# MadNLP/MadNLP.jl

Measured on NVIDIA H100. Metric: ipm_iters_per_sec, higher is better.
Workload: dtype f64

## Files before the change

### include/b200kkt.h

```cpp
#ifndef B200KKT_H
#define B200KKT_H

#include <stdint.h>

#ifdef __cplusplus
extern "C" {
#endif

#define B2_OK                 0
#define B2_ERR_INVALID        1
#define B2_ERR_CUDA           2
#define B2_ERR_SYMBOLIC       3
#define B2_ERR_FACTORIZATION  4
#define B2_ERR_SOLVE          5
#define B2_ERR_NO_DEVICE      6
#define B2_ERR_UNSUPPORTED    7

#define B2_ORDER_METIS_ND 0
#define B2_ORDER_MINDEG   1
#define B2_ORDER_NATURAL  2
#define B2_ORDER_USER     3

const char* b2_last_error(void);
int b2_version(void);
// ... 3 lines not shown
    int32_t ordering;
    int32_t nemin;
    double  relax_zeros;
    double  pivot_eps;
    int32_t use_cuda_graph;
    int32_t small_front_max;
    int32_t n_parts;
    int32_t part_rank;
    int32_t kkt_n_primal;
    int32_t fuse_max_fronts;
    int32_t dep_schedule;
    int32_t chain_merge_f;
    int32_t kkt_n_dual;
    int32_t dense_pivoting;
    int32_t sparse_pivoting;
    int32_t reserved[1];
} b2_options;

#define B2_DENSE_PIVOT_STATIC        0
#define B2_DENSE_PIVOT_BUNCH_KAUFMAN 1
#define B2_SPARSE_PIVOT_STATIC       0
#define B2_SPARSE_PIVOT_PAIRS        1

#define B2_PIVOT_1X1            0
#define B2_PIVOT_1X1_PERTURBED  1
#define B2_PIVOT_2X2_FIRST      2
#define B2_PIVOT_2X2_SECOND     3

int b2_options_default(b2_options* opt);

typedef struct b2_solver b2_solver;

typedef struct b2_stats {
    int64_t n, nnz_a, nnz_l, flops;
    int64_t n_supernodes, n_levels;
    int64_t max_front, n_small_fronts, n_big_fronts;
    int64_t factor_bytes, workspace_bytes;
    int64_t sep_rows;
    int64_t n_factor_launches, n_solve_launches;
    int64_t n_perturbed;
} b2_stats;

int b2_create(int32_t n, int64_t nnz, const int32_t* colptr_h, const int32_t* rowval_h,
              const double* nzval_d, const b2_options* opt, const int32_t* user_perm_h,
              b2_solver** out);
int b2_create_symbolic_only(int32_t n, int64_t nnz, const int32_t* colptr_h, const int32_t* rowval_h,
                            const b2_options* opt, const int32_t* user_perm_h, b2_solver** out);
int b2_destroy(b2_solver* s);
int b2_set_values_ptr(b2_solver* s, const double* nzval_d);
int b2_factorize(b2_solver* s, void* stream);
int b2_inertia(b2_solver* s, int64_t* num_pos, int64_t* num_zero, int64_t* num_neg, void* stream);
int b2_inertia_enqueue(b2_solver* s, void* stream);
int b2_inertia_fetch(b2_solver* s, int64_t* num_pos, int64_t* num_zero, int64_t* num_neg);
int b2_solve(b2_solver* s, double* x_d, int32_t nrhs, void* stream);
int b2_improve(b2_solver* s, int32_t* changed);
int b2_get_stats(b2_solver* s, b2_stats* st);
int b2_get_perm(b2_solver* s, int32_t* perm_h);

int b2_exchange_buffer(b2_solver* s, double** buf_d, int64_t* n_factor_doubles, int64_t* n_solve_doubles);
int b2_exchange_vector(b2_solver* s, double** buf_d, int64_t* n_doubles);
int b2_inertia_parts(b2_solver* s, int64_t* local_neg, int64_t* local_zero, int64_t* top_neg, int64_t* top_zero, void* stream);
int b2_factorize_local(b2_solver* s, void* stream);
int b2_factorize_top(b2_solver* s, void* stream);
int b2_solve_fwd_local(b2_solver* s, double* x_d, void* stream);
int b2_solve_top(b2_solver* s, double* x_d, void* stream);
int b2_solve_bwd_local(b2_solver* s, double* x_d, void* stream);
int b2_owned_mask(b2_solver* s, uint8_t* owned_h);

typedef struct b2_symbolic_sizes {
    int64_t n, n_supernodes, n_rows, n_children, n_rel, n_amap, n_levels, lval_size, cb_size;
} b2_symbolic_sizes;
int b2_symbolic_query(b2_solver* s, b2_symbolic_sizes* sz);
int b2_symbolic_export(b2_solver* s, int32_t* perm, int32_t* sn_first, int32_t* sn_parent, int32_t* sn_level,
                       int64_t* rows_ptr, int32_t* rows, int64_t* lp_off, int64_t* cb_off,
                       int64_t* rel_ptr, int32_t* rel, int64_t* amap_ptr, int64_t* amap_src, int64_t* amap_dst);
int b2_symbolic_owner(b2_solver* s, int32_t* owner);
int b2_symbolic_exchange(b2_solver* s, int64_t* cbv_off, int64_t* exch_cb, int64_t* exch_cbv);
int b2_debug_get_factor(b2_solver* s, double* lval_h, double* dvec_h);
int b2_symbolic_pairs(b2_solver* s, uint8_t* pair_start_h);
int b2_get_pivot_blocks(b2_solver* s, int8_t* kind_h, double* d_h, double* d_off_h);
int b2_debug_profile_front(b2_solver* s, int32_t sn, int32_t reps, int64_t* stamps_h);
int b2_debug_trace(b2_solver* s, uint64_t* stamps_h, int32_t* parent_h, int32_t* w_h, int32_t* f_h, int64_t capacity, int64_t* count);
int b2_debug_trace_solve(b2_solver* s, uint64_t* stamps_h, int64_t capacity, int64_t* count);

typedef struct b2d_solver b2d_solver;
int b2d_create(int32_t N, int32_t lda, const double* A_d, const b2_options* opt, b2d_solver** out);
int b2d_destroy(b2d_solver* s);
int b2d_debug_trace(b2d_solver* s, uint64_t* stamps_h, int64_t capacity, int64_t* count);
int b2d_factorize(b2d_solver* s, void* stream);
int b2d_inertia(b2d_solver* s, int64_t* num_pos, int64_t* num_zero, int64_t* num_neg, void* stream);
int b2d_inertia_enqueue(b2d_solver* s, void* stream);
int b2d_inertia_fetch(b2d_solver* s, int64_t* num_pos, int64_t* num_zero, int64_t* num_neg);
int b2d_solve(b2d_solver* s, double* x_d, int32_t nrhs, void* stream);
int b2d_get_pivots(b2d_solver* s, int32_t* ipiv_h, double* d_h, double* e_h);

int b2_coo_to_csc(int32_t m, int32_t n, int64_t nnz_coo, const int32_t* I_h, const int32_t* J_h,
                  int32_t* colptr_h, int32_t* rowval_h, int64_t* map_h, int64_t* nnz_csc);

int b2_coo_to_csc_device(int32_t m, int32_t n, int64_t nnz_coo, const int32_t* I_d, const int32_t* J_d,
                         int32_t* colptr_d, int32_t* rowval_d, int64_t* map_d, int64_t* nnz_csc, void* stream);

typedef struct b2_transfer_plan b2_transfer_plan;
int b2_transfer_plan_create(int64_t nnz_coo, int64_t nnz_csc, const int64_t* map_h, b2_transfer_plan** out);
int b2_transfer_plan_destroy(b2_transfer_plan* p);
int b2_transfer(b2_transfer_plan* p, double* dst_nz_d, const double* V_d, void* stream);

typedef struct b2_condensed_plan b2_condensed_plan;
int b2_condensed_symbolic(int32_t n, int32_t m,
                          const int32_t* H_colptr_h, const int32_t* H_rowval_h,
                          const int32_t* Jt_colptr_h, const int32_t* Jt_rowval_h,
                          b2_condensed_plan** out, int64_t* nnz_aug);
int b2_condensed_symbolic_device(int32_t n, int32_t m,
                                 const int32_t* H_colptr_d, const int32_t* H_rowval_d,
                                 const int32_t* Jt_colptr_d, const int32_t* Jt_rowval_d,
                                 b2_condensed_plan** out, int64_t* nnz_aug, void* stream);
int b2_condensed_pattern(b2_condensed_plan* p, int32_t* colptr_h, int32_t* rowval_h);
int b2_condensed_plan_sizes(b2_condensed_plan* p, int64_t* n_dptr, int64_t* n_hptr, int64_t* n_jptr);
int b2_condensed_plan_destroy(b2_condensed_plan* p);
int b2_condensed_assemble(b2_condensed_plan* p, double* aug_nz_d, const double* pr_diag_d,
                          const double* du_diag_d, const double* H_nz_d, const double* Jt_nz_d,
                          double* diag_buffer_d, void* stream);

int b2d_condensed_assemble(int32_t n, int32_t m, int32_t ns, int32_t n_eq,
                           const int64_t* ind_ineq_d, const int64_t* ind_eq_d,
                           const double* hess_d, const double* jac_d,
                           const double* pr_diag_d, const double* du_diag_d,
                           double* diag_buffer_d, double* aug_d, void* stream);

int b2d_aug_assemble(int32_t n, int32_t m, int32_t ns, const int64_t* ind_ineq_d,
                     const double* hess_d, const double* jac_d, const double* pr_diag_d,
                     const double* du_diag_d, const double* diag_hess_d, double* aug_d, void* stream);
int b2d_copy_diag(int32_t n, int32_t lda, const double* A_d, double* d_d, void* stream);

typedef struct b2d_ozaki_plan b2d_ozaki_plan;
int b2d_ozaki_plan_create(int32_t n, int32_t ns, b2d_ozaki_plan** out);
int b2d_ozaki_plan_destroy(b2d_ozaki_plan* p);
int b2d_condensed_assemble_ozaki(b2d_ozaki_plan* p, int32_t n, int32_t m, int32_t ns, int32_t n_eq,
                                 const int64_t* ind_ineq_d, const int64_t* ind_eq_d,
                                 const double* hess_d, const double* jac_d,
                                 const double* pr_diag_d, const double* du_diag_d,
                                 double* diag_buffer_d, double* aug_d, void* stream);
int b2d_ozaki_plan_status(b2d_ozaki_plan* p, int32_t* timed_out, void* stream);

int b2d_gemv_n(int32_t rows, int32_t cols, int32_t lda, const double* A_d, const double* x_d, double* y_d, double alpha, double beta, void* stream);
int b2d_gemv_t(int32_t rows, int32_t cols, int32_t lda, const double* A_d, const double* x_d, double* y_d, double alpha, double beta, void* stream);
int b2d_symv_lower(int32_t n, int32_t lda, const double* A_d, const double* x_d, double* y_d, double alpha, double beta, void* stream);

typedef struct b2_bounds b2_bounds;
typedef struct b2d_kkt b2d_kkt;
int b2d_kkt_create(int32_t n, int32_t m, int32_t ns, const int64_t* ind_ineq_h, b2d_kkt** out);
int b2d_kkt_destroy(b2d_kkt* k);
int b2d_kkt_solve_pre(b2d_kkt* k, b2_bounds* b, const double* jac_d, const double* pr_diag_d, const double* diag_buffer_d,
                      const double* l_diag_d, const double* u_diag_d, double* buffer_d, double* pd_buffer_d, double* w_d, void* stream);
int b2d_kkt_solve_post(b2d_kkt* k, b2_bounds* b, const double* jac_d, const double* pr_diag_d, const double* diag_buffer_d,
                       const double* l_lower_d, const double* u_lower_d, const double* l_diag_d, const double* u_diag_d,
                       const double* buffer_d, const double* pd_buffer_d, double* w_d, void* stream);
int b2d_kkt_mul(b2d_kkt* k, b2_bounds* b, const double* hess_d, const double* jac_d, const double* reg_d, const double* du_diag_d,
                const double* l_lower_d, const double* u_lower_d, const double* l_diag_d, const double* u_diag_d,
                double alpha, double beta, const double* x_d, double* w_d, void* stream);

typedef struct b2_bounds b2_bounds;
int b2_bounds_create(int64_t n_tot, int64_t nlb, int64_t nub, const int64_t* ind_lb_h, const int64_t* ind_ub_h,
                     b2_bounds** out);
int b2_bounds_destroy(b2_bounds* b);

int b2_set_aug_diagonal(b2_bounds* b, const double* reg_d, const double* l_lower_d, const double* l_diag_d,
// ... 307 lines not shown
```

### madnlp.jl_b200/capi.py

```python
from __future__ import annotations

import ctypes as C
import os

_HERE = os.path.dirname(os.path.abspath(__file__))
LIB_PATH = os.path.join(_HERE, "csrc", "libb200kkt.so")

B2_OK = 0
B2_ERR_INVALID, B2_ERR_CUDA, B2_ERR_SYMBOLIC, B2_ERR_FACTORIZATION, B2_ERR_SOLVE, B2_ERR_NO_DEVICE, B2_ERR_UNSUPPORTED = 1, 2, 3, 4, 5, 6, 7
ORDER_METIS_ND, ORDER_MINDEG, ORDER_NATURAL, ORDER_USER = 0, 1, 2, 3
QN_BFGS, QN_DAMPED_BFGS = 1, 2
B2_DENSE_PIVOT_STATIC, B2_DENSE_PIVOT_BUNCH_KAUFMAN = 0, 1
B2_SPARSE_PIVOT_STATIC, B2_SPARSE_PIVOT_PAIRS = 0, 1
B2_PIVOT_1X1, B2_PIVOT_1X1_PERTURBED, B2_PIVOT_2X2_FIRST, B2_PIVOT_2X2_SECOND = 0, 1, 2, 3
CURV_WXT, CURV_WXN, CURV_GN, CURV_TT, CURV_LHS, CURV_PASS, CURV_RESULT_LEN = 0, 1, 2, 3, 4, 5, 6
DUAL_INIT_NORM, DUAL_INIT_COPY, DUAL_INIT_RESULT_LEN = 0, 1, 2
QF_TAU, QF_NRM_PRIMAL, QF_NRM_DUAL, QF_MU_AVG, QF_SCAL_LEN = 0, 1, 2, 3, 4
QF_SIGMA, QF_MU, QF_N_EVAL, QF_N_GS_ITER, QF_TOL_EXIT, QF_TRACE, QF_MAX_GS_ITER = 0, 1, 2, 3, 4, 8, 64
KRYLOV_MAX_RESTART, KRYLOV_Y, KRYLOV_REC, KRYLOV_REC_LEN, KRYLOV_STATE_LEN = 16, 321, 344, 8, 352
KREC_EST, KREC_H, KREC_NORM_W, KREC_NORM_X, KREC_NORM_B, KREC_NORM_B2 = 0, 1, 2, 3, 4, 5


def qf_result_len(max_gs_iter):
    return QF_TRACE + 4 * (6 + max_gs_iter)
# ... 50 lines not shown


class InertiaSource(C.Structure):
    _fields_ = [("counters_d", C.c_void_p), ("n", C.c_int64), ("neg", C.c_int32 * 2), ("zero", C.c_int32 * 2), ("fail", C.c_int32),
                ("reserved", C.c_int32)]


class RefineRecord(C.Structure):
    _fields_ = [("ratio", C.c_double), ("norm_w", C.c_double), ("norm_x", C.c_double), ("norm_b", C.c_double), ("ir", C.c_int64),
                ("steps", C.c_int64), ("num_pos", C.c_int64), ("num_zero", C.c_int64), ("num_neg", C.c_int64), ("inertia_ok", C.c_int32),
                ("fail", C.c_int32), ("seq", C.c_int64)]


class InertiaSchedule(C.Structure):
    _fields_ = [(k, C.c_double) for k in ("first_hessian_perturbation", "min_hessian_perturbation", "max_hessian_perturbation",
                                          "perturb_inc_fact_first", "perturb_inc_fact", "perturb_dec_fact")]


TRIALS_ACCEPTED, TRIALS_FAILED, TRIALS_HANDOVER, TRIALS_FAULT = 1, 2, 3, 4


class InertiaRecord(C.Structure):
    _fields_ = [("status", C.c_int32), ("inertia_ok", C.c_int32), ("trials", C.c_int64), ("del_w", C.c_double),
                ("del_w_prev", C.c_double), ("del_c_prev", C.c_double), ("num_pos", C.c_int64), ("num_zero", C.c_int64),
                ("num_neg", C.c_int64), ("ir", C.c_int64), ("ratio", C.c_double), ("ir_total", C.c_int64), ("seq", C.c_int64)]


class SymbolicSizes(C.Structure):
    _fields_ = [(k, C.c_int64) for k in (
        "n", "n_supernodes", "n_rows", "n_children", "n_rel", "n_amap", "n_levels", "lval_size", "cb_size")]


def _load():
    if not os.path.exists(LIB_PATH):
        raise ImportError(
            f"{LIB_PATH} not found: build it with `python -c 'import __graft_entry__ as g; g.build()'` "
            f"(or `make -C madnlp.jl_b200/csrc`). The GPU KKT path has no CPU fallback.")
    return C.CDLL(LIB_PATH)


lib = _load()

_p = C.c_void_p
_i32, _i64, _f64 = C.c_int32, C.c_int64, C.c_double
_PP = C.POINTER(C.c_void_p)

PROTOTYPES = {
    "b2_last_error": (C.c_char_p, []),
    "b2_version": (C.c_int, []),
    "b2_device_count": (C.c_int, [C.POINTER(C.c_int)]),
    "b2_options_default": (C.c_int, [C.POINTER(Options)]),
    "b2_create": (C.c_int, [_i32, _i64, _p, _p, _p, C.POINTER(Options), _p, _PP]),
    "b2_create_symbolic_only": (C.c_int, [_i32, _i64, _p, _p, C.POINTER(Options), _p, _PP]),
    "b2_destroy": (C.c_int, [_p]),
    "b2_set_values_ptr": (C.c_int, [_p, _p]),
    "b2_factorize": (C.c_int, [_p, _p]),
    "b2_inertia": (C.c_int, [_p, C.POINTER(_i64), C.POINTER(_i64), C.POINTER(_i64), _p]),
    "b2_inertia_enqueue": (C.c_int, [_p, _p]),
    "b2_inertia_fetch": (C.c_int, [_p, C.POINTER(_i64), C.POINTER(_i64), C.POINTER(_i64)]),
    "b2_solve": (C.c_int, [_p, _p, _i32, _p]),
    "b2_improve": (C.c_int, [_p, C.POINTER(_i32)]),
    "b2_get_stats": (C.c_int, [_p, C.POINTER(Stats)]),
    "b2_get_perm": (C.c_int, [_p, _p]),
    "b2_exchange_buffer": (C.c_int, [_p, _PP, C.POINTER(_i64), C.POINTER(_i64)]),
    "b2_exchange_vector": (C.c_int, [_p, _PP, C.POINTER(_i64)]),
    "b2_inertia_parts": (C.c_int, [_p, C.POINTER(_i64), C.POINTER(_i64), C.POINTER(_i64), C.POINTER(_i64), _p]),
    "b2_factorize_local": (C.c_int, [_p, _p]),
    "b2_factorize_top": (C.c_int, [_p, _p]),
    "b2_solve_fwd_local": (C.c_int, [_p, _p, _p]),
    "b2_solve_top": (C.c_int, [_p, _p, _p]),
    "b2_solve_bwd_local": (C.c_int, [_p, _p, _p]),
    "b2_owned_mask": (C.c_int, [_p, _p]),
    "b2_symbolic_query": (C.c_int, [_p, C.POINTER(SymbolicSizes)]),
    "b2_symbolic_export": (C.c_int, [_p] + [_p] * 13),
    "b2_symbolic_owner": (C.c_int, [_p, _p]),
    "b2_symbolic_exchange": (C.c_int, [_p, _p, C.POINTER(_i64), C.POINTER(_i64)]),
    "b2_debug_get_factor": (C.c_int, [_p, _p, _p]),
    "b2_symbolic_pairs": (C.c_int, [_p, _p]),
    "b2_get_pivot_blocks": (C.c_int, [_p, _p, _p, _p]),
    "b2_debug_profile_front": (C.c_int, [_p, _i32, _i32, _p]),
    "b2d_debug_trace": (C.c_int, [_p, _p, _i64, C.POINTER(_i64)]),
    "b2_debug_trace": (C.c_int, [_p, _p, _p, _p, _p, _i64, C.POINTER(_i64)]),
    "b2_debug_trace_solve": (C.c_int, [_p, _p, _i64, C.POINTER(_i64)]),
    "b2d_create": (C.c_int, [_i32, _i32, _p, C.POINTER(Options), _PP]),
    "b2d_destroy": (C.c_int, [_p]),
    "b2d_factorize": (C.c_int, [_p, _p]),
    "b2d_inertia": (C.c_int, [_p, C.POINTER(_i64), C.POINTER(_i64), C.POINTER(_i64), _p]),
    "b2d_inertia_enqueue": (C.c_int, [_p, _p]),
    "b2d_inertia_fetch": (C.c_int, [_p, C.POINTER(_i64), C.POINTER(_i64), C.POINTER(_i64)]),
    "b2d_solve": (C.c_int, [_p, _p, _i32, _p]),
    "b2d_get_pivots": (C.c_int, [_p, _p, _p, _p]),
    "b2_condensed_symbolic_device": (C.c_int, [_i32, _i32, _p, _p, _p, _p, _PP, C.POINTER(_i64), _p]),
    "b2_coo_to_csc_device": (C.c_int, [_i32, _i32, _i64, _p, _p, _p, _p, _p, C.POINTER(_i64), _p]),
    "b2d_ozaki_plan_create": (C.c_int, [_i32, _i32, _PP]),
    "b2d_ozaki_plan_destroy": (C.c_int, [_p]),
    "b2d_condensed_assemble_ozaki": (C.c_int, [_p, _i32, _i32, _i32, _i32] + [_p] * 9),
    "b2d_ozaki_plan_status": (C.c_int, [_p, C.POINTER(_i32), _p]),
    "b2d_kkt_create": (C.c_int, [_i32, _i32, _i32, _p, _PP]),
    "b2d_kkt_destroy": (C.c_int, [_p]),
    "b2d_kkt_solve_pre": (C.c_int, [_p] * 10 + [_p]),
    "b2d_kkt_solve_post": (C.c_int, [_p] * 12 + [_p]),
    "b2d_kkt_mul": (C.c_int, [_p] * 10 + [_f64, _f64, _p, _p, _p]),
    "b2d_gemv_n": (C.c_int, [_i32, _i32, _i32, _p, _p, _p, _f64, _f64, _p]),
    "b2d_gemv_t": (C.c_int, [_i32, _i32, _i32, _p, _p, _p, _f64, _f64, _p]),
    "b2d_symv_lower": (C.c_int, [_i32, _i32, _p, _p, _p, _f64, _f64, _p]),
    "b2_coo_to_csc": (C.c_int, [_i32, _i32, _i64, _p, _p, _p, _p, _p, C.POINTER(_i64)]),
    "b2_transfer_plan_create": (C.c_int, [_i64, _i64, _p, _PP]),
    "b2_transfer_plan_destroy": (C.c_int, [_p]),
    "b2_transfer": (C.c_int, [_p, _p, _p, _p]),
    "b2_condensed_symbolic": (C.c_int, [_i32, _i32, _p, _p, _p, _p, _PP, C.POINTER(_i64)]),
    "b2_condensed_pattern": (C.c_int, [_p, _p, _p]),
    "b2_condensed_plan_sizes": (C.c_int, [_p, C.POINTER(_i64), C.POINTER(_i64), C.POINTER(_i64)]),
    "b2_condensed_plan_destroy": (C.c_int, [_p]),
    "b2_condensed_assemble": (C.c_int, [_p, _p, _p, _p, _p, _p, _p, _p]),
    "b2d_condensed_assemble": (C.c_int, [_i32, _i32, _i32, _i32, _p, _p, _p, _p, _p, _p, _p, _p, _p]),
    "b2d_aug_assemble": (C.c_int, [_i32, _i32, _i32] + [_p] * 8),
    "b2d_copy_diag": (C.c_int, [_i32, _i32, _p, _p, _p]),
    "b2_bounds_create": (C.c_int, [_i64, _i64, _i64, _p, _p, _PP]),
    "b2_bounds_destroy": (C.c_int, [_p]),
    "b2_set_aug_diagonal": (C.c_int, [_p, _p, _p, _p, _p, _p, _p, _p]),
    "b2_set_aug_diagonal_unreduced": (C.c_int, [_i64, _i64, _i64] + [_p] * 7),
    "b2_unreduced_solve_pre": (C.c_int, [_i64, _i64, _i64, _i64, _p, _p, _p, _p]),
    "b2_unreduced_solve_post": (C.c_int, [_i64, _i64, _i64, _i64, _p, _p, _p, _p]),
    "b2_regularize_diagonal": (C.c_int, [_i64, _i64, _f64, _f64, _p, _p, _p, _p]),
    "b2_reduce_rhs": (C.c_int, [_p, _i64, _p, _p, _p, _p]),
    "b2_finish_aug_solve": (C.c_int, [_p, _i64, _p, _p, _p, _p, _p, _p]),
    "b2_spmv_plan_create": (C.c_int, [_i32, _i32, _p, _p, _PP]),
    "b2_spmv_plan_destroy": (C.c_int, [_p]),
    "b2_spmv_n": (C.c_int, [_p, _p, _p, _p, _f64, _f64, _p]),
    "b2_spmv_t": (C.c_int, [_p, _p, _p, _p, _f64, _f64, _p]),
    "b2_spmv_symlower": (C.c_int, [_p, _p, _p, _p, _f64, _f64, _p]),
    "b2_kktmul": (C.c_int, [_p, _i64, _p, _p, _p, _p, _p, _p, _f64, _f64, _p, _p, _p]),
    "b2_condensed_solve_pre": (C.c_int, [_p, _p, _i64, _i64, _p, _p, _p, _p, _p, _p, _p, _p]),
    "b2_condensed_solve_post": (C.c_int, [_p, _p, _i64, _i64, _p, _p, _p, _p, _p, _p, _p, _p, _p, _p]),
    "b2_condensed_kkt_mul": (C.c_int, [_p, _p, _p, _i64, _i64, _p, _p, _p, _p, _p, _p, _p, _p, _f64, _f64, _p, _p, _p]),
    "b2_condensed_kkt_mul_norm": (C.c_int, [_p, _p, _p, _i64, _i64, _p, _p, _p, _p, _p, _p, _p, _p, _f64, _f64, _p, _p, _p, _p]),
    "b2_condensed_refine_pre": (C.c_int, [_p, _p, _i64, _i64, _p, _p, _p, _p, _p, _p, _p, _p, _p]),
    "b2_condensed_solve_post_update": (C.c_int, [_p, _p, _i64, _i64, _p, _p, _p, _p, _p, _p, _p, _p, _p, _p, _p, _p]),
    "b2_condensed_kkt_mul_norm_y": (C.c_int, [_p, _p, _p, _i64, _i64, _p, _p, _p, _p, _p, _p, _p, _p, _f64, _f64, _p, _p, _p, _p, _p]),
    "b2_get_alpha_max": (C.c_int, [_p, _p, _p, _p, _p, _f64, _p, _p]),
    "b2_get_alpha_z": (C.c_int, [_p, _p, _p, _p, _p, _f64, _p, _p]),
    "b2_get_varphi": (C.c_int, [_p, _f64, _p, _p, _p, _f64, _p, _p]),
    "b2_get_varphi_d": (C.c_int, [_p, _p, _p, _p, _p, _p, _f64, _p, _p]),
    "b2_get_inf_du": (C.c_int, [_p, _p, _p, _p, _p, _f64, _p, _p]),
    "b2_get_inf_compl": (C.c_int, [_p, _p, _p, _p, _p, _p, _f64, _f64, _p, _p]),
    "b2_get_average_complementarity": (C.c_int, [_p, _p, _p, _p, _p, _p, _p, _p]),
    "b2_get_min_complementarity": (C.c_int, [_p, _p, _p, _p, _p, _p, _p, _p]),
    "b2_get_rel_search_norm": (C.c_int, [_p, _i64, _p, _p, _p, _p]),
    "b2_get_sd": (C.c_int, [_p, _i64, _p, _p, _p, _f64, _p, _p]),
    "b2_get_sc": (C.c_int, [_p, _p, _p, _f64, _p, _p]),
    "b2_set_aug_rhs": (C.c_int, [_p, _i64, _p, _p, _p, _p, _p, _p, _p, _p, _f64, _p, _p]),
    "b2_set_g_ifr": (C.c_int, [_i64, _p, _p, _p, _p, _p, _f64, _p, _p]),
    "b2_set_aug_rhs_ifr": (C.c_int, [_i64, _i64, _i64, _i64, _p, _p, _p]),
    "b2_mul_hess_blk_tail": (C.c_int, [_p, _i64, _i32] + [_p] * 9 + [_f64, _p, _p]),
    "b2_rr_init": (C.c_int, [_p, _i64, _p, _p, _f64, _f64] + [_p] * 10 + [_p]),
    "b2_set_aug_rr": (C.c_int, [_p, _i64, _f64, _f64, _f64] + [_p] * 16 + [_p]),
    "b2_set_aug_rhs_rr": (C.c_int, [_p, _i64] + [_p] * 13 + [_f64, _f64, _p, _p]),
    "b2_finish_aug_solve_rr": (C.c_int, [_i64] + [_p] * 6 + [_f64, _f64] + [_p] * 4 + [_p]),
    "b2_set_f_rr": (C.c_int, [_i64, _f64, _p, _p, _p, _p, _p]),
    "b2_reset_bound_dual": (C.c_int, [_i64, _p, _p, _f64, _f64, _p]),
    "b2_reset_bound_dual_lu": (C.c_int, [_p] + [_p] * 5 + [_f64, _f64, _p]),
    "b2_adjust_boundary": (C.c_int, [_p, _p, _p, _p, _f64, _p]),
    "b2_get_theta": (C.c_int, [_p, _i64, _p, _p, _p]),
    "b2_get_theta_r": (C.c_int, [_p, _i64, _p, _p, _p, _p, _p]),
    "b2_get_inf_pr_r": (C.c_int, [_p, _i64, _p, _p, _p, _p, _p]),
    "b2_get_obj_val_r": (C.c_int, [_p, _i64] + [_p] * 5 + [_f64, _f64, _p, _p]),
# ... 129 lines not shown
```

### madnlp.jl_b200/csrc/sparse_ldl.cu

```cuda
#include <algorithm>
#include <cstdlib>
#include <cstring>
#include <stdexcept>
#include <vector>

#include "analysis.hpp"
#include "common.cuh"
#include "front_kernels.cuh"
#include "bigfactor_kernels.cuh"
#include "solve_kernels.cuh"
#include "warp_kernels.cuh"
#include "bigsolve_kernels.cuh"
#include "densesolve_kernels.cuh"
#include "dense_bk.cuh"

using namespace b2;

namespace {

struct WarpLaunch {
    int n_cta = 0, cta_ptr_off = 0, stage_off_off = 0, stage_cnt_off = 0;
    int nw = 1;
    int maxf = 0;
};
// ... 319 lines not shown
}

template <int NR>
constexpr size_t solve_block_smem() {
    return sizeof(double) * std::max<size_t>((size_t)4 * SolveSmem<1, NR>::doubles, (size_t)SolveSmem<2, NR>::doubles);
}
template <int NR>
const void* solve_block_kernel(bool pairs) {
    return pairs ? (const void*)k_solve_dep_block<NR, true> : (const void*)k_solve_dep_block<NR, false>;
}

template <int NR>
void enqueue_solve_block(b2_solver* s, double* x, int ncol, cudaStream_t st) {
    const Phase& P = s->phase[0];
    SolveArgs a = solve_args(s);
    a.perm = s->d_perm.p;
    a.x = x;
    const int64_t nr = s->cbv_off[s->S.nsuper];
    a.up = s->d_bslots.p;
    a.down = s->d_bslots.p + NR * nr;
    a.ypiv = s->d_bslots.p + 2 * NR * nr;
    DepSched ds;
    ds.grp_type = s->d_sched.p + P.dep_type_off; ds.grp_ptr = s->d_sched.p + P.dep_ptr_off; ds.tasks = s->d_sched.p + P.dep_tasks_off;
    ds.ngroup = P.dep_ngroup;
    const int w = NR == 2 ? 0 : NR == 4 ? 1 : 2;
    auto kern = s->pairs ? k_solve_dep_block<NR, true> : k_solve_dep_block<NR, false>;
    kern<<<P.sol_grid_blk[w], 128, solve_block_smem<NR>(), st>>>(a, s->d_childrec.p, ds, s->d_counters.p + 4, s->d_flags.p + s->S.nsuper + 1,
                                                                 s->S.n, ncol, s->d_bslots.p, (int64_t)s->d_bslots.n, s->d_dsub.p);
}

template <int NR>
cudaError_t set_level_block_attrs() {
    const void* k[] = {(const void*)k_fwd_warp2_block<1, SOLVE_FUSED_TEAMS, NR>, (const void*)k_bwd_warp2_block<1, SOLVE_FUSED_TEAMS, NR>,
                       (const void*)k_fwd_warp2_block<1, FW_WARPS, NR>, (const void*)k_bwd_warp2_block<1, FW_WARPS, NR>,
                       (const void*)k_fwd_warp2_block<2, 1, NR>, (const void*)k_bwd_warp2_block<2, 1, NR>,
                       (const void*)k_bs_head_block<NR>, (const void*)k_bs_fwd_block<NR>, (const void*)k_bs_bwd_block<NR>};
    for (const void* f : k) {
        cudaError_t e = cudaFuncSetAttribute(f, cudaFuncAttributeMaxDynamicSharedMemorySize, 100 * 1024);
        if (e != cudaSuccess) return e;
    }
    return cudaSuccess;
}

int set_smem_attrs() {
    B2_CUDA(cudaFuncSetAttribute(k_front_smem<512>, cudaFuncAttributeMaxDynamicSharedMemorySize, 227 * 1024));
    B2_CUDA(cudaFuncSetAttribute(k_factor_warp<1>, cudaFuncAttributeMaxDynamicSharedMemorySize, 160 * 1024));
    B2_CUDA(cudaFuncSetAttribute(k_factor_warp<2>, cudaFuncAttributeMaxDynamicSharedMemorySize, 160 * 1024));
    B2_CUDA(cudaFuncSetAttribute(k_factor_dep, cudaFuncAttributeMaxDynamicSharedMemorySize, 160 * 1024));
    B2_CUDA(cudaFuncSetAttribute(k_factor_dep_pairs, cudaFuncAttributeMaxDynamicSharedMemorySize, 160 * 1024));
    B2_CUDA(cudaFuncSetAttribute(k_fwd_warp2<1>, cudaFuncAttributeMaxDynamicSharedMemorySize, 100 * 1024));
    B2_CUDA(cudaFuncSetAttribute(k_bwd_warp2<1>, cudaFuncAttributeMaxDynamicSharedMemorySize, 100 * 1024));
    B2_CUDA(cudaFuncSetAttribute((k_fwd_warp2<1, SOLVE_FUSED_TEAMS>), cudaFuncAttributeMaxDynamicSharedMemorySize, 100 * 1024));
    B2_CUDA(cudaFuncSetAttribute((k_bwd_warp2<1, SOLVE_FUSED_TEAMS>), cudaFuncAttributeMaxDynamicSharedMemorySize, 100 * 1024));
    B2_CUDA(cudaFuncSetAttribute(k_fwd_warp2<2>, cudaFuncAttributeMaxDynamicSharedMemorySize, 100 * 1024));
    B2_CUDA(cudaFuncSetAttribute(k_bwd_warp2<2>, cudaFuncAttributeMaxDynamicSharedMemorySize, 100 * 1024));
    B2_CUDA(cudaFuncSetAttribute(k_solve_dep, cudaFuncAttributeMaxDynamicSharedMemorySize, 100 * 1024));
    B2_CUDA(cudaFuncSetAttribute(k_solve_dep_pairs, cudaFuncAttributeMaxDynamicSharedMemorySize, 100 * 1024));
    B2_CUDA(set_level_block_attrs<2>());
    B2_CUDA(set_level_block_attrs<4>());
    B2_CUDA(set_level_block_attrs<8>());
    for (bool pairs : {false, true}) {
        B2_CUDA(cudaFuncSetAttribute(solve_block_kernel<2>(pairs), cudaFuncAttributeMaxDynamicSharedMemorySize, 100 * 1024));
        B2_CUDA(cudaFuncSetAttribute(solve_block_kernel<4>(pairs), cudaFuncAttributeMaxDynamicSharedMemorySize, 100 * 1024));
        B2_CUDA(cudaFuncSetAttribute(solve_block_kernel<8>(pairs), cudaFuncAttributeMaxDynamicSharedMemorySize, 100 * 1024));
    }
    B2_CUDA(cudaFuncSetAttribute(k_big_inv, cudaFuncAttributeMaxDynamicSharedMemorySize, 160 * 1024));
    return B2_OK;
}

template <typename Fn>
int capture(b2_solver* s, cudaGraphExec_t* out, Fn fn) {
    if (*out) { cudaGraphExecDestroy(*out); *out = nullptr; }
    cudaGraph_t g = nullptr;
    B2_CUDA(cudaStreamBeginCapture(s->cap_stream, cudaStreamCaptureModeThreadLocal));
    fn(s->cap_stream);
    cudaError_t e = cudaStreamEndCapture(s->cap_stream, &g);
    if (e != cudaSuccess) return cuda_fail(e, "cudaStreamEndCapture", __FILE__, __LINE__);
    e = cudaGraphInstantiate(out, g, 0);
    cudaGraphDestroy(g);
    if (e != cudaSuccess) return cuda_fail(e, "cudaGraphInstantiate", __FILE__, __LINE__);
    return B2_OK;
}

void build_schedule(b2_solver* s) {
    const Symbolic& S = s->S;
    const int ns = S.nsuper;
    const int rank = std::max(0, s->opt.part_rank);
    const int smax = s->opt.small_front_max;
    const int wmax = std::min(W_MAX, smax);
    const int w1max = std::min(32, smax);
    const int fuse_max = s->opt.fuse_max_fronts;
    std::vector<int32_t> sched;
    auto fdim = [&](int sn, int& w, int& f) {
        w = S.sn_first[sn + 1] - S.sn_first[sn];
        f = (int)(S.rows_ptr[sn + 1] - S.rows_ptr[sn]);
    };
    auto emit_warp_launch = [&](const std::vector<std::vector<std::vector<int32_t>>>& ctas, int nw) {
        WarpLaunch L;
        L.nw = nw;
        L.n_cta = (int)ctas.size();
        std::vector<int32_t> cta_ptr(1, 0), st_off, st_cnt;
        for (const auto& stages : ctas) {
            for (const auto& fr : stages) {
                st_off.push_back((int32_t)sched.size());
                st_cnt.push_back((int32_t)fr.size());
                for (int32_t sn : fr) {
                    int w, f; fdim(sn, w, f);
                    L.maxf = std::max(L.maxf, f);
                    sched.push_back(sn);
                }
            }
            cta_ptr.push_back((int32_t)st_off.size());
        }
        L.cta_ptr_off = (int)sched.size(); sched.insert(sched.end(), cta_ptr.begin(), cta_ptr.end());
        L.stage_off_off = (int)sched.size(); sched.insert(sched.end(), st_off.begin(), st_off.end());
        L.stage_cnt_off = (int)sched.size(); sched.insert(sched.end(), st_cnt.begin(), st_cnt.end());
        return L;
    };
    for (int ph = 0; ph < 2; ++ph) {
        Phase& P = s->phase[ph];
        P.lev.clear(); P.fused = WarpLaunch(); P.n_fused_fronts = 0; P.dep_ngroup = 0; P.sol_grid = 0;
        std::vector<char> mine(ns, 0);
        for (int sn = 0; sn < ns; ++sn) mine[sn] = (ph == 0) ? (S.owner[sn] == rank) : (S.owner[sn] == -1);
        if ((s->opt.dep_schedule & 1) && s->opt.n_parts <= 1 && wmax > 32) {
            bool all_team = true;
            int cntm = 0;
            for (int sn = 0; sn < ns && all_team; ++sn) if (mine[sn]) { int w, f; fdim(sn, w, f); all_team = f <= wmax; ++cntm; }
            if (all_team && cntm > 0) {
                std::vector<int32_t> order;
                for (int l = 0; l < S.nlevels; ++l)
                    for (int q = S.level_ptr[l]; q < S.level_ptr[l + 1]; ++q) if (mine[S.level_sn[q]]) order.push_back(S.level_sn[q]);
                std::vector<int32_t> gtype, gptr(1, 0), tasks;
                size_t k = 0;
                while (k < order.size()) {
                    int w, f; fdim(order[k], w, f);
                    if (f > 32) {
                        gtype.push_back(2); tasks.push_back(order[k]); ++k;
                        P.dep_maxf2 = std::max(P.dep_maxf2, f);
                    } else {
                        gtype.push_back(1);
                        int c = 0;
                        while (k < order.size() && c < FW_WARPS) {
                            int w2, f2; fdim(order[k], w2, f2);
                            if (f2 > 32) break;
                            tasks.push_back(order[k]); P.dep_maxf1 = std::max(P.dep_maxf1, f2); ++k; ++c;
                        }
                    }
                    gptr.push_back((int32_t)tasks.size());
                }
                P.dep_ngroup = (int)gtype.size();
                P.dep_type_off = (int)sched.size(); sched.insert(sched.end(), gtype.begin(), gtype.end());
                P.dep_ptr_off = (int)sched.size(); sched.insert(sched.end(), gptr.begin(), gptr.end());
                P.dep_tasks_off = (int)sched.size(); sched.insert(sched.end(), tasks.begin(), tasks.end());
            }
        }
        std::vector<int32_t> cnt(ns, 0);
        std::vector<char> okw(ns, 0);
        for (int sn = 0; sn < ns; ++sn) {
            if (!mine[sn]) continue;
            int w, f; fdim(sn, w, f);
            bool ok = f <= w1max;
            int c = 1;
            for (int q = S.child_ptr[sn]; q < S.child_ptr[sn + 1]; ++q) {
                const int ch = S.child_idx[q];
                if (!mine[ch]) { continue; }
                ok = ok && okw[ch];
                c += cnt[ch];
            }
            cnt[sn] = c;
            okw[sn] = ok && fuse_max > 0 && c <= fuse_max;
        }
        std::vector<int32_t> root_of(ns, -1);
        std::vector<int32_t> roots;
        for (int sn = ns - 1; sn >= 0; --sn) {
            if (!mine[sn] || !okw[sn]) continue;
            const int p = S.sn_parent[sn];
            if (p >= 0 && mine[p] && okw[p]) root_of[sn] = root_of[p];
            else { root_of[sn] = sn; roots.push_back(sn); }
        }
        std::reverse(roots.begin(), roots.end());
        if (!roots.empty()) {
            std::vector<int32_t> ridx(ns, -1);
            for (size_t k = 0; k < roots.size(); ++k) ridx[roots[k]] = (int32_t)k;
            std::vector<std::vector<std::vector<int32_t>>> ctas(roots.size());
            for (int sn = 0; sn < ns; ++sn) {
                if (root_of[sn] < 0) continue;
                auto& stages = ctas[ridx[root_of[sn]]];
                const int lv = S.sn_level[sn];
                if ((int)stages.size() <= lv) stages.resize(lv + 1);
                stages[lv].push_back(sn);
                P.n_fused_fronts++;
            }
            for (auto& stages : ctas) {
                std::vector<std::vector<int32_t>> t;
                for (auto& v : stages) if (!v.empty()) t.push_back(std::move(v));
                stages.swap(t);
            }
            std::stable_sort(ctas.begin(), ctas.end(), [](const auto& a, const auto& b) {
                size_t na = 0, nb = 0;
                for (auto& v : a) na += v.size();
                for (auto& v : b) nb += v.size();
                return na > nb;
            });
            P.fused = emit_warp_launch(ctas, 1);
        }
        std::vector<int32_t> ulev(ns, -1);
        int nul = 0;
        for (int sn = 0; sn < ns; ++sn) {
            if (!mine[sn] || root_of[sn] >= 0) continue;
            int lv = 0;
            for (int q = S.child_ptr[sn]; q < S.child_ptr[sn + 1]; ++q) {
                const int ch = S.child_idx[q];
                if (mine[ch] && root_of[ch] < 0) lv = std::max(lv, ulev[ch] + 1);
            }
// ... 563 lines not shown
    return B2_OK;
}

int b2_exchange_buffer(b2_solver* s, double** buf_d, int64_t* n_factor_doubles, int64_t* n_solve_doubles) {
    if (!s || s->symbolic_only) return B2_ERR_INVALID;
    if (buf_d) *buf_d = s->d_ws.p;
    if (n_factor_doubles) *n_factor_doubles = s->S.exch_cb;
    if (n_solve_doubles) *n_solve_doubles = s->exch_cbv;
    return B2_OK;
}

int b2_exchange_vector(b2_solver* s, double** buf_d, int64_t* n_doubles) {
    if (!s || s->symbolic_only) return B2_ERR_INVALID;
    if (buf_d) *buf_d = s->d_cbv.p;
    if (n_doubles) *n_doubles = s->exch_cbv;
    return B2_OK;
}

int b2_owned_mask(b2_solver* s, uint8_t* owned_h) {
    if (!s || !owned_h) return B2_ERR_INVALID;
    std::memcpy(owned_h, s->owned_mask.data(), s->owned_mask.size());
    return B2_OK;
}

int b2_symbolic_query(b2_solver* s, b2_symbolic_sizes* sz) {
    if (!s || !sz) return B2_ERR_INVALID;
    const Symbolic& S = s->S;
    sz->n = S.n; sz->n_supernodes = S.nsuper; sz->n_rows = (int64_t)S.rows.size();
    sz->n_children = (int64_t)S.child_idx.size(); sz->n_rel = (int64_t)S.rel.size();
    sz->n_amap = (int64_t)S.amap_src.size(); sz->n_levels = S.nlevels;
    sz->lval_size = S.lp_off[S.nsuper]; sz->cb_size = S.cb_off[S.nsuper];
    return B2_OK;
}

int b2_symbolic_export(b2_solver* s, int32_t* perm, int32_t* sn_first, int32_t* sn_parent, int32_t* sn_level,
                       int64_t* rows_ptr, int32_t* rows, int64_t* lp_off, int64_t* cb_off,
                       int64_t* rel_ptr, int32_t* rel, int64_t* amap_ptr, int64_t* amap_src, int64_t* amap_dst) {
    if (!s) return B2_ERR_INVALID;
    const Symbolic& S = s->S;
    auto cp = [](auto* dst, const auto& v) { if (dst) std::memcpy(dst, v.data(), v.size() * sizeof(v[0])); };
    cp(perm, S.perm); cp(sn_first, S.sn_first); cp(sn_parent, S.sn_parent); cp(sn_level, S.sn_level);
    cp(rows_ptr, S.rows_ptr); cp(rows, S.rows); cp(lp_off, S.lp_off); cp(cb_off, S.cb_off);
    cp(rel_ptr, S.rel_ptr); cp(rel, S.rel); cp(amap_ptr, S.amap_ptr); cp(amap_src, S.amap_src); cp(amap_dst, S.amap_dst);
    return B2_OK;
}

int b2_debug_profile_front(b2_solver* s, int32_t sn, int32_t reps, int64_t* stamps_h) {
    if (!s || s->symbolic_only || sn < 0 || sn >= s->S.nsuper || reps < 1 || reps > 64) return B2_ERR_INVALID;
    const int f = (int)(s->S.rows_ptr[sn + 1] - s->S.rows_ptr[sn]);
    if (f > W_MAX) { set_error("b2_debug_profile_front: front is not team-class"); return B2_ERR_INVALID; }
    DevBuf<long long> prof;
    B2_CUDA(prof.alloc(8 * reps));
    FactorArgs a = factor_args(s);
    a.counters += 2;
    if (f <= 32) {
        B2_CUDA(cudaFuncSetAttribute(k_factor_team_profile<1>, cudaFuncAttributeMaxDynamicSharedMemorySize, 160 * 1024));
        k_factor_team_profile<1><<<1, 32, (size_t)TeamSmem<1>::doubles(f) * sizeof(double)>>>(a, s->d_childrec.p, sn, f, prof.p, reps);
    } else {
        B2_CUDA(cudaFuncSetAttribute(k_factor_team_profile<2>, cudaFuncAttributeMaxDynamicSharedMemorySize, 160 * 1024));
        k_factor_team_profile<2><<<1, 64, (size_t)TeamSmem<2>::doubles(f) * sizeof(double)>>>(a, s->d_childrec.p, sn, f, prof.p, reps);
    }
    B2_CUDA(cudaDeviceSynchronize());
    B2_CUDA(cudaMemcpy(stamps_h, prof.p, 8 * reps * sizeof(long long), cudaMemcpyDeviceToHost));
    return B2_OK;
}

int b2_debug_trace(b2_solver* s, uint64_t* stamps_h, int32_t* parent_h, int32_t* w_h, int32_t* f_h, int64_t capacity, int64_t* count) {
    if (!s || !count) { set_error("b2_debug_trace: invalid argument"); return B2_ERR_INVALID; }
    const int64_t ns = s->S.nsuper;
    *count = ns;
    if (capacity < ns) return B2_OK;
    for (int64_t i = 0; i < ns; ++i) {
        if (parent_h) parent_h[i] = s->S.sn_parent[i];
        const int w = s->S.sn_first[i + 1] - s->S.sn_first[i];
        if (w_h) w_h[i] = w;
        if (f_h) f_h[i] = (int32_t)(s->S.rows_ptr[i + 1] - s->S.rows_ptr[i]);
    }
    if (stamps_h && s->d_ftrace.p) {
        B2_CUDA(cudaDeviceSynchronize());
        B2_CUDA(cudaMemcpy(stamps_h, s->d_ftrace.p, s->d_ftrace.bytes(), cudaMemcpyDeviceToHost));
    } else if (stamps_h) {
        std::memset(stamps_h, 0, (size_t)3 * ns * sizeof(uint64_t));
    }
    return B2_OK;
}

int b2_debug_trace_solve(b2_solver* s, uint64_t* stamps_h, int64_t capacity, int64_t* count) {
    if (!s || !count) { set_error("b2_debug_trace_solve: invalid argument"); return B2_ERR_INVALID; }
    *count = s->d_strace.p ? (int64_t)6 * s->S.nsuper : 0;
    if (stamps_h && *count && capacity >= *count) {
        B2_CUDA(cudaDeviceSynchronize());
        B2_CUDA(cudaMemcpy(stamps_h, s->d_strace.p, s->d_strace.bytes(), cudaMemcpyDeviceToHost));
    }
    return B2_OK;
}

int b2_debug_get_factor(b2_solver* s, double* lval_h, double* dvec_h) {
    if (!s || s->symbolic_only) return B2_ERR_INVALID;
    B2_CUDA(cudaDeviceSynchronize());
    if (lval_h) B2_CUDA(cudaMemcpy(lval_h, s->d_L.p, (size_t)s->S.lp_off[s->S.nsuper] * sizeof(double), cudaMemcpyDeviceToHost));
    if (dvec_h) B2_CUDA(cudaMemcpy(dvec_h, s->d_dvec.p, s->d_dvec.bytes(), cudaMemcpyDeviceToHost));
    return B2_OK;
}

int b2_symbolic_pairs(b2_solver* s, uint8_t* pair_start_h) {
    if (!s || !pair_start_h) return B2_ERR_INVALID;
    std::memcpy(pair_start_h, s->S.pair_start.data(), (size_t)s->S.n);
    return B2_OK;
}

int b2_get_pivot_blocks(b2_solver* s, int8_t* kind_h, double* d_h, double* d_off_h) {
    if (!s || s->symbolic_only) { set_error("b2_get_pivot_blocks: solver has no device state"); return B2_ERR_INVALID; }
    if (!s->pairs) { set_error("b2_get_pivot_blocks: the handle pivots statically (opt.sparse_pivoting = 0)"); return B2_ERR_INVALID; }
    if (!s->factorized) { set_error("b2_get_pivot_blocks: not factorized"); return B2_ERR_FACTORIZATION; }
    B2_CUDA(cudaDeviceSynchronize());
    if (kind_h) B2_CUDA(cudaMemcpy(kind_h, s->d_pkind.p, s->d_pkind.bytes(), cudaMemcpyDeviceToHost));
    if (d_h) B2_CUDA(cudaMemcpy(d_h, s->d_dvec.p, s->d_dvec.bytes(), cudaMemcpyDeviceToHost));
    if (d_off_h) B2_CUDA(cudaMemcpy(d_off_h, s->d_dsub.p, s->d_dsub.bytes(), cudaMemcpyDeviceToHost));
    return B2_OK;
}

int b2_symbolic_exchange(b2_solver* s, int64_t* cbv_off, int64_t* exch_cb, int64_t* exch_cbv) {
    if (!s) return B2_ERR_INVALID;
    if (cbv_off) std::memcpy(cbv_off, s->cbv_off.data(), s->cbv_off.size() * sizeof(int64_t));
    if (exch_cb) *exch_cb = s->S.exch_cb;
    if (exch_cbv) *exch_cbv = s->exch_cbv;
    return B2_OK;
}

int b2_symbolic_owner(b2_solver* s, int32_t* owner) {
    if (!s || !owner) return B2_ERR_INVALID;
    std::memcpy(owner, s->S.owner.data(), s->S.owner.size() * sizeof(int32_t));
    return B2_OK;
}

}

struct b2d_solver {
    int32_t N = 0, lda = 0;
    const double* A_d = nullptr;
    b2_options opt;
    DevBuf<double> fact, dvec, linv, side, flow;
    DevBuf<int32_t> tilecnt;
    DevBuf<unsigned long long> trace;
    cudaStream_t aux_stream = nullptr;
    cudaStream_t side_stream = nullptr;
    std::vector<cudaEvent_t> ev_pool;
    size_t ev_next = 0;
    DevBuf<int64_t> linv_off;
    DevBuf<FrontDesc> desc;
    DevBuf<int32_t> list, counters;
    int32_t* h_counters = nullptr;
    cudaGraphExec_t g_factor = nullptr;
    cudaStream_t cap_stream = nullptr;
    bool factorized = false;
    bool bunch_kaufman = false;
    DenseBK bk;
    ~b2d_solver() {
        if (g_factor) cudaGraphExecDestroy(g_factor);
        for (auto e : ev_pool) cudaEventDestroy(e);
        if (aux_stream) cudaStreamDestroy(aux_stream);
        if (side_stream) cudaStreamDestroy(side_stream);
        if (cap_stream) cudaStreamDestroy(cap_stream);
        if (h_counters) cudaFreeHost(h_counters);
    }
};
// ... 276 lines not shown
```

### madnlp.jl_b200/csrc/warp_kernels.cuh

```cuda
#pragma once
#include "common.cuh"
#include "front_kernels.cuh"
#include "ptx.cuh"
#include "solve_kernels.cuh"

namespace b2 {

constexpr int FW_WARPS = 4;

struct ChildRec {
    int64_t cb_off;
    int64_t rel_off;
    int64_t cbv_off;
    int32_t rc;
    int32_t sn;
};
static_assert(sizeof(ChildRec) == 32, "ChildRec must be 32 bytes");

struct WarpSched {
    const int32_t* cta_ptr;
    const int32_t* stage_off;
    const int32_t* stage_cnt;
    const int32_t* list;
};

#define B2_STAMP(idx) do { if (prof) { team_sync<NW>(team); if (tid == 0) prof[idx] = clock64(); } } while (0)

template <int NW>
__device__ __forceinline__ void team_sync(int team) {
    if (NW == 1) __syncwarp();
    else asm volatile("bar.sync %0, %1;" ::"r"(team + 1), "r"(NW * 32) : "memory");
}

template <int NW>
__device__ __forceinline__ void team_arrive(int team, int warp, int parity) {
    static_assert(NW <= 2, "split barrier is written for one- and two-warp teams");
    if (NW == 2) asm volatile("bar.arrive %0, 64;" ::"r"(3 + team * 4 + warp * 2 + parity) : "memory");
}
template <int NW>
__device__ __forceinline__ void team_wait(int team, int warp, int parity) {
    if (NW == 1) __syncwarp();
    else asm volatile("bar.sync %0, 64;" ::"r"(3 + team * 4 + (warp ^ 1) * 2 + parity) : "memory");
}

constexpr int MAXC = 8;
template <int NW>
struct TeamSmem {
    static constexpr int FMAX = 32 * NW;
    static constexpr int STAGE = (NW == 1) ? 1024 : 4096;
    static __host__ __device__ int fsize(int maxf) { return (maxf * maxf + 1) & ~1; }
    static __host__ __device__ int doubles(int maxf) {
        return fsize(maxf) + 4 * (FMAX + 4) + (MAXC * FMAX) / 2 + MAXC * 4 + STAGE;
    }
};

constexpr unsigned DEP_SPIN_MAX = 1u << 24, DEP_SPIN_SLEEP_NS = 32;
__device__ __forceinline__ void flag_wait(const int* flag, int* err, int want = 1) {
    if (!bounded_spin<DEP_SPIN_MAX, DEP_SPIN_SLEEP_NS>(err, [&](unsigned) { return ld_acquire(flag) == want; })) __threadfence();
}

__device__ __forceinline__ void slot_put(double* p, double v) {
    const unsigned long long b = (unsigned long long)__double_as_longlong(v);
    st_relaxed_b64(p, b == SLOT_EMPTY ? CANON_NAN : b);
}
template <int K>
__device__ __forceinline__ void slot_take(double* const (&p)[K], unsigned need, double (&v)[K], int* err) {
    unsigned long long b[K];
#pragma unroll
    for (int c = 0; c < K; ++c) b[c] = (need >> c & 1u) ? ld_relaxed_b64(p[c]) : 0ull;
    unsigned it = 0;
    for (;;) {
        unsigned pend = 0;
#pragma unroll
        for (int c = 0; c < K; ++c) pend |= ((need >> c & 1u) && b[c] == SLOT_EMPTY) ? 1u << c : 0u;
        if (!pend) break;
        if (++it >= DEP_SPIN_MAX) {
            atomicExch(err, 1);
            break;
        }
        __nanosleep(DEP_SPIN_SLEEP_NS);
#pragma unroll
        for (int c = 0; c < K; ++c) if (pend >> c & 1u) b[c] = ld_relaxed_b64(p[c]);
    }
#pragma unroll
    for (int c = 0; c < K; ++c) {
        v[c] = __longlong_as_double((long long)b[c]);
        if ((need >> c & 1u) && b[c] != SLOT_EMPTY) st_relaxed_b64(p[c], SLOT_EMPTY);
    }
}

template <int NR>
__device__ __forceinline__ void slot_put_block(double* p, const double (&v)[NR]) {
    if constexpr (NR == 1) {
        slot_put(p, v[0]);
    } else {
        static_assert(NR % 2 == 0, "block slots are accessed in 16-byte pairs");
        unsigned long long b[NR];
#pragma unroll
        for (int q = 0; q < NR; ++q) {
            b[q] = (unsigned long long)__double_as_longlong(v[q]);
            b[q] = b[q] == SLOT_EMPTY ? CANON_NAN : b[q];
        }
#pragma unroll
        for (int q = 0; q < NR; q += 2) st_relaxed_v2_b64(p + q, b[q], b[q + 1]);
    }
}
template <int K, int NR>
__device__ __forceinline__ void slot_take_block(double* const (&p)[K], unsigned need, double (&v)[K][NR], int* err) {
    if constexpr (NR == 1) {
        double u[K];
        slot_take(p, need, u, err);
#pragma unroll
        for (int c = 0; c < K; ++c) v[c][0] = u[c];
    } else {
        static_assert(NR % 2 == 0, "block slots are accessed in 16-byte pairs");
        unsigned long long b[K][NR];
#pragma unroll
        for (int c = 0; c < K; ++c)
#pragma unroll
            for (int q = 0; q < NR; q += 2) {
                if (need >> c & 1u) ld_relaxed_v2_b64(p[c] + q, b[c][q], b[c][q + 1]);
                else b[c][q] = b[c][q + 1] = 0ull;
            }
        unsigned it = 0, pend;
        for (;;) {
            pend = 0;
#pragma unroll
            for (int c = 0; c < K; ++c) {
                bool empty = false;
#pragma unroll
                for (int q = 0; q < NR; ++q) empty |= b[c][q] == SLOT_EMPTY;
                pend |= ((need >> c & 1u) && empty) ? 1u << c : 0u;
            }
            if (!pend) break;
            if (++it >= DEP_SPIN_MAX) {
                atomicExch(err, 1);
                break;
            }
            __nanosleep(DEP_SPIN_SLEEP_NS);
#pragma unroll
            for (int c = 0; c < K; ++c)
                if (pend >> c & 1u)
// ... 41 lines not shown
    if constexpr (NP > 1) { pending_pair<NW, 1>(av, lp, up); B2_TIE(r, av[1], av[2]); }
    e = fma(-dk, r, 1.0);
    if constexpr (NP > 2) { pending_pair<NW, 2>(av, lp, up); B2_TIE(e, av[3], av[4]); }
    r = fma(r, e, r);
    if constexpr (NP > 3) { pending_pair<NW, 3>(av, lp, up); B2_TIE(r, av[5], av[6]); }
    e = fma(-dk, r, 1.0);
    if constexpr (NP > 4) { pending_pair<NW, 4>(av, lp, up); B2_TIE(e, av[7], av[8]); }
    r = fma(r, e, r);
    if constexpr (NP > 5) { pending_pair<NW, 5>(av, lp, up); B2_TIE(r, av[9], av[10]); }
    double l = av[0] * r;
    if constexpr (NP > 6) { pending_pair<NW, 6>(av, lp, up); B2_TIE(l, av[11], av[12]); }
    double nx = fma(-l, u0, a1);
    double* dst = c.nb + (c.tid - c.k);
    if (NW == 1) {
        if (c.tid > c.k) *dst = nx;
    } else {
        asm volatile("{\n\t.reg .pred p;\n\tsetp.gt.s32 p, %2, %3;\n\t@p st.shared.f64 [%0], %1;\n\tbar.arrive %4, 64;\n\t}"
                     ::"r"(smem_u32(dst)), "d"(nx), "r"(c.tid), "r"(c.k),
                       "r"(3 + c.team * 4 + (c.tid >> 5) * 2 + ((c.k + 1) & 1)));
    }
    if (c.tid < c.f) c.Fk[c.tid] = (c.tid == c.k) ? dk : l;
    av[0] = nx;
    PendingRange<NW, 7, NP>::run(av, lp, up);
    lp = l;
}

struct PairArgs {
    const unsigned long long* mask = nullptr;
    double* dsub = nullptr;
    int8_t* kind = nullptr;
};
constexpr double PAIR_ALPHA = 0.6403882032022076;

template <int NW, bool DEP = false, bool PAIRS = false>
__device__ __forceinline__ void front_factor_team(const FactorArgs& a, const ChildRec* childrec, int s, double* sm_team,
                                                  int tid, int team, int maxf, int& nneg, int& npert, long long* prof = nullptr,
                                                  int* done = nullptr, int* err = nullptr, PairArgs pa = PairArgs()) {
    constexpr int FMAX = 32 * NW, TEAM = 32 * NW, STAGE = TeamSmem<NW>::STAGE;
    double* F = sm_team;
    constexpr int CBS = FMAX + 4;
    double* colbuf = F + TeamSmem<NW>::fsize(maxf);
    int* relst = (int*)(colbuf + 4 * CBS);
    ChildRec* recs = (ChildRec*)(relst + MAXC * FMAX);
    double* stage = (double*)(recs + MAXC);
    B2_STAMP(0);
    if (a.ftrace && tid == 0) a.ftrace[3 * (size_t)s] = global_ns();
    const FrontDesc d = a.desc[s];
    const int f = d.f, w = d.w, r = f - w;
    B2_STAMP(1);
    for (int i = tid; i < f * f; i += TEAM) F[i] = 0.0;
    for (int i = tid; i < 4 * CBS; i += TEAM) colbuf[i] = 0.0;
    team_sync<NW>(team);
    B2_STAMP(2);
    {
        const int32_t* src = a.amap_src + d.amap_off;
        const int32_t* dst = a.amap_dst + d.amap_off;
        for (int t0 = 0; t0 < d.amap_cnt; t0 += 4 * TEAM) {
            int sd[4], dd[4]; double v[4];
#pragma unroll
            for (int u = 0; u < 4; ++u) {
                const int t = t0 + tid + u * TEAM;
                sd[u] = (t < d.amap_cnt) ? src[t] : -1;
                dd[u] = (t < d.amap_cnt) ? dst[t] : 0;
            }
#pragma unroll
            for (int u = 0; u < 4; ++u) v[u] = (sd[u] >= 0) ? __ldg(a.A + sd[u]) : 0.0;
#pragma unroll
            for (int u = 0; u < 4; ++u) if (sd[u] >= 0) F[dd[u]] = v[u];
        }
    }
    team_sync<NW>(team);
    B2_STAMP(3);
    int* nready_sh = relst + FMAX - 1;
    for (int c0 = 0; c0 < d.nchild;) {
        const int cb0 = (c0 / MAXC) * MAXC;
        const int ro = c0 - cb0;
        if (ro == 0) {
            if (tid < min(MAXC, d.nchild - cb0)) recs[tid] = childrec[d.child_off + cb0 + tid];
            team_sync<NW>(team);
        }
        int nrec = min(MAXC, d.nchild - cb0) - ro;
        if (DEP) {
            if (tid < 32) {
                if (tid == 0) flag_wait(done + recs[ro].sn, err);
                __syncwarp();
                int v = (tid == 0) ? 1 : 0;
                if (tid > 0 && tid < nrec) v = ld_acquire(done + recs[ro + tid].sn);
                const unsigned m = __ballot_sync(0xffffffffu, v != 0);
                if (tid == 0) *nready_sh = __ffs(~m) - 1;
            }
            team_sync<NW>(team);
            nrec = *nready_sh;
        }
        const ChildRec* rrec = recs + ro;
        int nc = 0, tot = 0;
        while (nc < nrec) {
            const int sz = (rrec[nc].rc * rrec[nc].rc + 1) & ~1;
            if (nc > 0 && tot + sz > STAGE) break;
            tot += sz; ++nc;
        }
        int off = 0;
        for (int c = 0; c < nc; ++c) {
            const int rc = rrec[c].rc;
            const double* CB = a.ws + rrec[c].cb_off;
            const int sz = (rc * rc + 1) & ~1;
            if (DEP) { for (int e = 2 * tid; e < sz; e += 2 * TEAM) cp_async16_cg(stage + off + e, CB + e); }
            else { for (int e = tid; e < rc * rc; e += TEAM) cp_async8(stage + off + e, CB + e); }
            if (tid < rc) cp_async4(relst + c * FMAX + tid, a.rel + rrec[c].rel_off + tid);
            off += sz;
        }
        cp_async_wait_all();
        team_sync<NW>(team);
        off = 0;
        for (int c = 0; c < nc; ++c) {
            const int rc = rrec[c].rc;
            const int* rl = relst + c * FMAX;
            const double* cs = stage + off;
            if (tid < rc) {
                const int ri = rl[tid];
                for (int j0 = 0; j0 <= tid; j0 += 8) {
                    double v[8], g[8]; int ix[8];
#pragma unroll
                    for (int u = 0; u < 8; ++u) { const int j = j0 + u; ix[u] = (j <= tid) ? ri + rl[j] * f : -1; }
#pragma unroll
                    for (int u = 0; u < 8; ++u) { const int j = j0 + u; v[u] = (ix[u] >= 0) ? cs[j * rc + tid] : 0.0; g[u] = (ix[u] >= 0) ? F[ix[u]] : 0.0; }
#pragma unroll
                    for (int u = 0; u < 8; ++u) if (ix[u] >= 0) F[ix[u]] = g[u] + v[u];
                }
            }
            team_sync<NW>(team);
            off += (rc * rc + 1) & ~1;
        }
        c0 += nc;
    }
    B2_STAMP(4);
    if (a.ftrace && tid == 0) a.ftrace[3 * (size_t)s + 1] = global_ns();
    double av[FMAX + 1];
    if constexpr (PAIRS) {
        const unsigned long long pm = pa.mask[s];
        double* u1 = colbuf;
        double* u2 = colbuf + CBS;
        for (int k = 0; k < w;) {
            team_sync<NW>(team);
            const double av_ = F[k + k * f];
            bool two = false;
            double b_ = 0.0, c_ = 0.0;
            if ((pm >> k) & 1ull) {
                b_ = F[k + 1 + k * f];
                c_ = F[(k + 1) * (f + 1)];
                const double t = fabs(b_);
                two = fabs(av_) < PAIR_ALPHA * t && (av_ / t) * c_ - t < 0.0;
            }
            if (!two) {
                const bool tiny = !(fabs(av_) >= a.eps), neg = av_ < 0.0;
                const double dk = tiny ? (neg ? -a.eps : a.eps) : av_;
                npert += (tid == 0 && tiny) ? 1 : 0;
                nneg += (tid == 0 && !tiny && neg) ? 1 : 0;
                if (tid > k && tid < f) u1[tid] = F[tid + k * f];
                team_sync<NW>(team);
                if (tid > k && tid < f) {
                    const double l = u1[tid] / dk;
                    for (int j = k + 1; j <= tid; ++j) F[tid + j * f] = fma(-l, u1[j], F[tid + j * f]);
                    F[tid + k * f] = l;
                }
                if (tid == 0) {
                    F[k + k * f] = dk;
                    pa.kind[d.col0 + k] = tiny ? 1 : 0;
                    pa.dsub[d.col0 + k] = 0.0;
                }
                k += 1;
            } else {
// ... 835 lines not shown
```

Measured before the change: 1852.

## Order dependent-schedule tasks by subtree depth and poll child flags warp-wide

The task order for the dependency-driven team schedule now sorts supernodes by depth within the owned subtree, deepest first, with level as the tie-breaker, instead of plain level order. The intent is that tasks whose children finish earliest are dispatched first, which should cut spin-waiting on dependency flags. The child-readiness check also changes: the whole warp now polls all pending child flags together in each spin iteration, instead of lane 0 spinning on the first child and then sampling the rest once. A debug export of the new order is added, and polling from every lane adds more memory traffic while spinning.

```diff
diff --git a/include/b200kkt.h b/include/b200kkt.h
--- a/include/b200kkt.h
+++ b/include/b200kkt.h
@@ -109,6 +109,7 @@
 int b2_debug_profile_front(b2_solver* s, int32_t sn, int32_t reps, int64_t* stamps_h);
 int b2_debug_trace(b2_solver* s, uint64_t* stamps_h, int32_t* parent_h, int32_t* w_h, int32_t* f_h, int64_t capacity, int64_t* count);
 int b2_debug_trace_solve(b2_solver* s, uint64_t* stamps_h, int64_t capacity, int64_t* count);
+int b2_debug_dep_order(b2_solver* s, int32_t* order_h, int64_t capacity, int64_t* count);
 
 typedef struct b2d_solver b2d_solver;
 int b2d_create(int32_t N, int32_t lda, const double* A_d, const b2_options* opt, b2d_solver** out);
diff --git a/madnlp.jl_b200/capi.py b/madnlp.jl_b200/capi.py
--- a/madnlp.jl_b200/capi.py
+++ b/madnlp.jl_b200/capi.py
@@ -156,6 +156,7 @@
     "b2d_debug_trace": (C.c_int, [_p, _p, _i64, C.POINTER(_i64)]),
     "b2_debug_trace": (C.c_int, [_p, _p, _p, _p, _p, _i64, C.POINTER(_i64)]),
     "b2_debug_trace_solve": (C.c_int, [_p, _p, _i64, C.POINTER(_i64)]),
+    "b2_debug_dep_order": (C.c_int, [_p, _p, _i64, C.POINTER(_i64)]),
     "b2d_create": (C.c_int, [_i32, _i32, _p, C.POINTER(Options), _PP]),
     "b2d_destroy": (C.c_int, [_p]),
     "b2d_factorize": (C.c_int, [_p, _p]),
diff --git a/madnlp.jl_b200/csrc/sparse_ldl.cu b/madnlp.jl_b200/csrc/sparse_ldl.cu
--- a/madnlp.jl_b200/csrc/sparse_ldl.cu
+++ b/madnlp.jl_b200/csrc/sparse_ldl.cu
@@ -425,6 +425,20 @@
     return B2_OK;
 }
 
+std::vector<int32_t> dep_ticket_order(const Symbolic& S, const std::vector<char>& mine) {
+    const int ns = S.nsuper;
+    std::vector<int32_t> depth(ns, 0), order;
+    for (int sn = ns - 1; sn >= 0; --sn) {
+        const int p = S.sn_parent[sn];
+        depth[sn] = (p >= 0 && mine[p]) ? depth[p] + 1 : 0;
+    }
+    for (int sn = 0; sn < ns; ++sn) if (mine[sn]) order.push_back(sn);
+    std::stable_sort(order.begin(), order.end(), [&](int32_t x, int32_t y) {
+        return depth[x] != depth[y] ? depth[x] > depth[y] : S.sn_level[x] < S.sn_level[y];
+    });
+    return order;
+}
+
 void build_schedule(b2_solver* s) {
     const Symbolic& S = s->S;
     const int ns = S.nsuper;
@@ -470,9 +484,7 @@
             int cntm = 0;
             for (int sn = 0; sn < ns && all_team; ++sn) if (mine[sn]) { int w, f; fdim(sn, w, f); all_team = f <= wmax; ++cntm; }
             if (all_team && cntm > 0) {
-                std::vector<int32_t> order;
-                for (int l = 0; l < S.nlevels; ++l)
-                    for (int q = S.level_ptr[l]; q < S.level_ptr[l + 1]; ++q) if (mine[S.level_sn[q]]) order.push_back(S.level_sn[q]);
+                const std::vector<int32_t> order = dep_ticket_order(S, mine);
                 std::vector<int32_t> gtype, gptr(1, 0), tasks;
                 size_t k = 0;
                 while (k < order.size()) {
@@ -1202,6 +1214,17 @@
     } else if (stamps_h) {
         std::memset(stamps_h, 0, (size_t)3 * ns * sizeof(uint64_t));
     }
+    return B2_OK;
+}
+
+int b2_debug_dep_order(b2_solver* s, int32_t* order_h, int64_t capacity, int64_t* count) {
+    if (!s || !count) { set_error("b2_debug_dep_order: invalid argument"); return B2_ERR_INVALID; }
+    const int rank = std::max(0, s->opt.part_rank);
+    std::vector<char> mine(s->S.nsuper);
+    for (int sn = 0; sn < s->S.nsuper; ++sn) mine[sn] = s->S.owner[sn] == rank;
+    const std::vector<int32_t> order = dep_ticket_order(s->S, mine);
+    *count = (int64_t)order.size();
+    if (order_h && capacity >= *count) std::copy(order.begin(), order.end(), order_h);
     return B2_OK;
 }
 
diff --git a/madnlp.jl_b200/csrc/warp_kernels.cuh b/madnlp.jl_b200/csrc/warp_kernels.cuh
--- a/madnlp.jl_b200/csrc/warp_kernels.cuh
+++ b/madnlp.jl_b200/csrc/warp_kernels.cuh
@@ -55,9 +55,6 @@
 };
 
 constexpr unsigned DEP_SPIN_MAX = 1u << 24, DEP_SPIN_SLEEP_NS = 32;
-__device__ __forceinline__ void flag_wait(const int* flag, int* err, int want = 1) {
-    if (!bounded_spin<DEP_SPIN_MAX, DEP_SPIN_SLEEP_NS>(err, [&](unsigned) { return ld_acquire(flag) == want; })) __threadfence();
-}
 
 __device__ __forceinline__ void slot_put(double* p, double v) {
     const unsigned long long b = (unsigned long long)__double_as_longlong(v);
@@ -265,11 +262,20 @@
         int nrec = min(MAXC, d.nchild - cb0) - ro;
         if (DEP) {
             if (tid < 32) {
-                if (tid == 0) flag_wait(done + recs[ro].sn, err);
-                __syncwarp();
-                int v = (tid == 0) ? 1 : 0;
-                if (tid > 0 && tid < nrec) v = ld_acquire(done + recs[ro + tid].sn);
-                const unsigned m = __ballot_sync(0xffffffffu, v != 0);
+                const int* fl = done + recs[ro + (tid < nrec ? tid : 0)].sn;
+                unsigned m, it = 0;
+                for (;;) {
+                    const int v = (tid < nrec) ? ld_acquire(fl) : 0;
+                    m = __ballot_sync(0xffffffffu, v != 0);
+                    if (m & 1u) break;
+                    if (++it >= DEP_SPIN_MAX) {
+                        if (tid == 0) atomicExch(err, 1);
+                        __threadfence();
+                        m = 1u;
+                        break;
+                    }
+                    __nanosleep(DEP_SPIN_SLEEP_NS);
+                }
                 if (tid == 0) *nready_sh = __ffs(~m) - 1;
             }
             team_sync<NW>(team);
```

New measurement: 1999 (median of 6 runs). 8.0% higher.
